# olivesgatech/R3D

Hardware: AMD Instinct MI355X
Metric: training clips/sec (RGB+Depth fusion, DARai) at 1/2/4/8 GPUs; effective-rank match (higher is better)
Workload: dtype f32 (depth products: bf16x3 split on the bf16 matrix cores, fp32 accumulate)

## Files before the change

include/r3d_hip.h:

```cpp
#ifndef R3D_HIP_H
#define R3D_HIP_H

#include <stdint.h>

#ifdef __cplusplus
extern "C" {
#endif

#define R3D_ABI_VERSION 2

#define R3D_OK 0
#define R3D_EINVAL (-1)
#define R3D_EALIGN (-2)
#define R3D_ENORCCL (-3)
#define R3D_ERCCL_BASE (-100)

int r3d_abi_version(void);
int r3d_build_info(char* buf, int cap);

int r3d_allreduce_flat(float* buf, int64_t count, void* comm, void* stream);

#define R3D_GEMM_NT 0
#define R3D_GEMM_NN 1
#define R3D_GEMM_TN 2
// ... 256 lines not shown
    const float* w_head; const float* b_head; int n_head;
    float* t3; float* m3; float* r3; float* tgtF; float* mF; float* rF; float* out; int ld_out; int H;
    const float* seg; int ld_seg; const int64_t* past_label; const int64_t* target; const float* target_dur;
    int B, S, Q, K, pad_idx, exclude_idx; const float* dur_den; float grad_scale;
    float* d_seg; int ld_dseg; float* d_out; int ld_dout; float* loss_out; int64_t* counts; int64_t* tick_a; int64_t* tick_b;
    const uint8_t* drop; float drop_scale; float* dx; float* dx2; float* wsF; float* ws3;
    int defer_finalize;
} r3d_tail_losses_args;
int r3d_decoder_tail_losses_supported(int H, int n_head, int Q, int rows);
int r3d_decoder_tail_losses(const r3d_tail_losses_args* a, float* ws, void* stream);

typedef struct r3d_decoder_chain_args {
    const float* caq; const float* cakv; const int64_t* key_label; float* p_ca; const uint8_t* drop_ca; float* ca_o;
    const float* wo; const float* bo; const uint8_t* drop_d2; const float* t1; float* t2_pre; const float* g2; const float* be2;
    float* t2; float* m2; float* r2; const float* w1; const float* b1; const uint8_t* drop_ff; float* ff1;
    const float* w2; const float* b2; const uint8_t* drop_d3; float* t3_pre;
    const float* d_t3pre; const float* d_ff2; float* d_ff1; float* d_t2pre; float* d_cap; float* d_cao; float* d_caq;
    float* d_cakv; float* part_d2;
    float drop_scale;
    int32_t pad_idx, B, S, H, Q, heads, phases;
    uint64_t* timeline;
    const uint16_t* pl_wo; const uint16_t* pl_w1; const uint16_t* pl_w2; const uint16_t* pl_w2_t; const uint16_t* pl_w1_t;
    const uint16_t* pl_wo_t;
} r3d_decoder_chain_args;
int r3d_decoder_chain_supported(int H, int Q, int heads, int S);
int r3d_decoder_chain(const r3d_decoder_chain_args* d, const r3d_tail_losses_args* tail, float* ws, void* stream);

int r3d_adamw_flat(float* p, const float* g, float* m, float* v, int64_t n, const float* lr, const int64_t* step,
                   float beta1, float beta2, float eps, float weight_decay, float grad_scale, void* stream);
int r3d_adamw_flat_dropout(float* p, const float* g, float* m, float* v, int64_t n, const float* lr, const int64_t* step,
                           float beta1, float beta2, float eps, float weight_decay, float grad_scale, uint8_t* mask,
                           int64_t n_mask, float p_drop, uint64_t seed, const int64_t* offset, void* stream);
typedef struct r3d_loss_finalize_job {
    const float* part; int32_t B, S, Q, has_seg;
    const float* dur_den;
    float* loss_out; int64_t* counts;
    double* acc_loss; int64_t* acc_counts;
} r3d_loss_finalize_job;
int r3d_losses_finalize(const r3d_loss_finalize_job* job, void* stream);
int r3d_adamw_flat_fin(float* p, const float* g, float* m, float* v, int64_t n, const float* lr, const int64_t* step,
                       float beta1, float beta2, float eps, float weight_decay, float grad_scale,
                       const r3d_loss_finalize_job* fin, void* stream);
int r3d_adamw_flat_dropout_fin(float* p, const float* g, float* m, float* v, int64_t n, const float* lr, const int64_t* step,
                               float beta1, float beta2, float eps, float weight_decay, float grad_scale, uint8_t* mask,
                               int64_t n_mask, float p_drop, uint64_t seed, const int64_t* offset,
                               const r3d_loss_finalize_job* fin, void* stream);
int r3d_adamw_2d(float* p, const float* g, float* m, float* v, int rows, int cols, int ld, const float* lr,
                 const int64_t* step, float beta1, float beta2, float eps, float weight_decay, float grad_scale, void* stream);
// ... 53 lines not shown
```

r3d_amd/_lib.py:

```python
import ctypes as C
import os

HERE = os.path.dirname(os.path.abspath(__file__))
LIB_PATH = os.path.join(HERE, "_build", "libr3d_hip.so")
ABI_VERSION = 2

c_float_p = C.c_void_p


class GemmDesc(C.Structure):
    _fields_ = [
        ("A", C.c_void_p), ("B", C.c_void_p), ("C", C.c_void_p),
        ("layout", C.c_int32), ("M", C.c_int32), ("N", C.c_int32), ("K", C.c_int32),
        ("lda", C.c_int32), ("ldb", C.c_int32), ("ldc", C.c_int32),
        ("a_add", C.c_void_p), ("a_add_mod", C.c_int32), ("a_add_ld", C.c_int32), ("a_row_xor", C.c_int32),
        ("b_add", C.c_void_p), ("b_add_mod", C.c_int32), ("b_add_ld", C.c_int32),
        ("bias", C.c_void_p),
        ("pre_out", C.c_void_p), ("ldpre", C.c_int32),
        ("act", C.c_int32),
        ("drop_mask", C.c_void_p), ("lddrop", C.c_int32), ("drop_scale", C.c_float),
        ("aux", C.c_void_p), ("ldaux", C.c_int32), ("mul", C.c_int32),
        ("res1", C.c_void_p), ("ldr1", C.c_int32),
        ("res2", C.c_void_p), ("ldr2", C.c_int32),
        ("alpha", C.c_float), ("accumulate", C.c_int32),
# ... 45 lines not shown


class PlaneJob(C.Structure):
    _fields_ = [("src", C.c_void_p), ("dst", C.c_void_p), ("ld", C.c_int32), ("N", C.c_int32), ("K", C.c_int32),
                ("transposed", C.c_int32), ("first_block", C.c_int32), ("pad_", C.c_int32)]


class FuserChainBwdArgs(C.Structure):
    _PTRS = ("d_cakv d_seg d_extra wkv wseg x3 mf rf gf w2 u w1 x1 m2 r2 g2 wproj wv x0 m1 r1 g1n drop_x0 m_rgb m_dep rgb "
             "dep_pre mean_d rstd_d lnd_g lnd_b d_fused d_x3 d_u d_h2 d_x1 d_v d_h1 d_rgb_pre d_dep_pre part_nf part_n2 "
             "part_n1 part_dep d_caq d_t1_res wq t1_pre m1d r1d g1d drop_d1 w_out sa_qkv p_sa drop_sa w_in caqin t1pre_out "
             "sap sao saqkv sain part_d1").split()
    _PLANES = "pl_wkv_t pl_wseg_t pl_w2_t pl_w1_t pl_wproj_t pl_wv_t".split()
    _fields_ = ([(n, C.c_void_p) for n in _PTRS] + [("drop_scale", C.c_float)] +
                [(n, C.c_int32) for n in "N S K H add_xres B Q heads".split()] + [("timeline", C.c_void_p)] +
                [(n, C.c_void_p) for n in _PLANES])


class DecoderChainArgs(C.Structure):
    _PTRS = ("caq cakv key_label p_ca drop_ca ca_o wo bo drop_d2 t1 t2_pre g2 be2 t2 m2 r2 w1 b1 drop_ff ff1 w2 b2 drop_d3 "
             "t3_pre d_t3pre d_ff2 d_ff1 d_t2pre d_cap d_cao d_caq d_cakv part_d2").split()
    _fields_ = ([(n, C.c_void_p) for n in _PTRS] + [("drop_scale", C.c_float)] +
                [(n, C.c_int32) for n in "pad_idx B S H Q heads phases".split()] + [("timeline", C.c_void_p)] +
                [(n, C.c_void_p) for n in "pl_wo pl_w1 pl_w2 pl_w2_t pl_w1_t pl_wo_t".split()])


class MhaJob(C.Structure):
    _fields_ = [("q", C.c_void_p), ("ldq", C.c_int32), ("k", C.c_void_p), ("ldk", C.c_int32), ("v", C.c_void_p),
                ("ldv", C.c_int32), ("key_padding_mask", C.c_void_p), ("key_label", C.c_void_p), ("pad_idx", C.c_int32),
                ("probs", C.c_void_p), ("drop_mask", C.c_void_p), ("drop_scale", C.c_float), ("o", C.c_void_p),
                ("ldo", C.c_int32), ("B", C.c_int32), ("heads", C.c_int32), ("Lq", C.c_int32), ("Lk", C.c_int32),
                ("dh", C.c_int32)]


class MhaBwdJob(C.Structure):
    _fields_ = [("q", C.c_void_p), ("ldq", C.c_int32), ("k", C.c_void_p), ("ldk", C.c_int32), ("v", C.c_void_p),
                ("ldv", C.c_int32), ("probs", C.c_void_p), ("drop_mask", C.c_void_p), ("drop_scale", C.c_float),
                ("d_o", C.c_void_p), ("lddo", C.c_int32), ("dq", C.c_void_p), ("lddq", C.c_int32), ("dk", C.c_void_p),
                ("lddk", C.c_int32), ("dv", C.c_void_p), ("lddv", C.c_int32), ("B", C.c_int32), ("heads", C.c_int32),
                ("Lq", C.c_int32), ("Lk", C.c_int32), ("dh", C.c_int32)]


class RowsumJob(C.Structure):
    _fields_ = [("src1", C.c_void_p), ("src2", C.c_void_p), ("dst", C.c_void_p), ("ld1", C.c_int32), ("ld2", C.c_int32),
                ("ldd", C.c_int32), ("rows", C.c_int32), ("cols", C.c_int32), ("mod", C.c_int32)]


# ... 36 lines not shown
    "r3d_build_info": ([C.c_char_p, _I], C.c_int),
    "r3d_allreduce_flat": ([_P, _L, _P, _P], C.c_int),
    "r3d_gemm_f32": ([C.POINTER(GemmDesc), _P], C.c_int),
    "r3d_splitk_reduce": ([C.POINTER(GemmDesc), _P], C.c_int),
    "r3d_gemm_partial_floats": ([C.c_int32, C.c_int32, C.c_int32], C.c_int64),
    "r3d_gemm_plan": ([C.POINTER(GemmDesc)], C.c_int),
    "r3d_gemm_grouped_prepare": ([C.POINTER(GemmDesc), _I, _I, C.POINTER(C.c_int32)], C.c_int),
    "r3d_gemm_grouped_launch": ([_P, _P, C.POINTER(C.c_int32), _I, _I, _I, _I, _P], C.c_int),
    "r3d_gemm_ln_supported": ([_I, _I, _I], C.c_int),
    "r3d_gemm_ln_fwd": ([_P, _I, _I, _P], C.c_int),
    "r3d_fuser_chain_supported": ([_I, _I, _I, _I, _I, _I], C.c_int),
    "r3d_fuser_chain_fwd": ([_P, _P], C.c_int),
    "r3d_fuser_chain_bwd": ([_P, _P], C.c_int),
    "r3d_weight_plane_elems": ([_I, _I], C.c_int64),
    "r3d_weight_planes": ([_P, _I, _I, _P], C.c_int),
    "r3d_token_exchange3_fwd": ([_P, _P, _P, _P, _P, _F, _P, _I, _I, _P], C.c_int),
    "r3d_token_exchange3_bwd": ([_P, _P, _P, _F, _P, _P, _P, _I, _I, _P], C.c_int),
    "r3d_attn3_fwd": ([_P, _P, _P, _I, _I, _I, _P], C.c_int),
    "r3d_attn3_bwd": ([_P, _P, _P, _I, _I, _I, _P], C.c_int),
    "r3d_triple_mean_fwd": ([_P, _P, _I, _I, _P], C.c_int),
    "r3d_triple_mean_bwd": ([_P, _P, _I, _I, _P], C.c_int),
    "r3d_decoder_chain_supported": ([_I, _I, _I, _I], C.c_int),
    "r3d_decoder_chain": ([_P, _P, _P, _P], C.c_int),
    "r3d_gemm_ln_mha_supported": ([_I, _I, _I, _I], C.c_int),
    "r3d_gemm_ln_mha_fwd": ([_P, _I, _I, _P, _P], C.c_int),
    "r3d_layernorm_fwd_multi": ([_P, _I, _P], C.c_int),
    "r3d_layernorm_bwd_multi": ([_P, _I, _P], C.c_int),
    "r3d_layernorm_bwd_multi_mha": ([_P, _I, _P, _P], C.c_int),
    "r3d_layernorm_bwd_finalize_batched": ([_P, _I, _I, _P], C.c_int),
    "r3d_layernorm_fwd": ([_P, _I, _I, _P, _P, _P, _P, _P, _I, _P, _P, _P, _I, _I, _I, _P], C.c_int),
    "r3d_layernorm_bwd_ws_floats": ([_I, _I], C.c_int64),
    "r3d_add_rowbcast": ([_P, _I, _P, _I, _I, _P, _I, _I, _I, _P], C.c_int),
    "r3d_layernorm_bwd": ([_P, _I, _I, _P, _I, _P, _I, _P, _P, _P, _P, _I, _P, _I, _P, _I, _P, _I, _P, _I, _P, _I, _F,
                           _P, _P, _P, _I, _I, _I, _P], C.c_int),
    "r3d_layernorm_bwd_finalize": ([_P, _I, _I, _P, _P, _P], C.c_int),
    "r3d_colsum_ws_floats": ([_I, _I], C.c_int64),
    "r3d_colsum": ([_P, _I, _I, _I, _P, _P, _I, _P], C.c_int),
    "r3d_rowmod_sum": ([_P, _I, _I, _I, _I, _P, _I, _I, _P], C.c_int),
    "r3d_rowmod_sum_batched": ([_P, _I, _I, _I, _P], C.c_int),
    "r3d_tick": ([_P, _P, _P], C.c_int),
    "r3d_colabssum": ([_P, _I, _I, _I, _P, _P], C.c_int),
    "r3d_token_select": ([_P, _P, _D, _I, _I, _I, _P, _P, _P, _P], C.c_int),
    "r3d_token_exchange_fwd": ([_P, _P, _P, _P, _P, _P, _F, _I, _I, _P], C.c_int),
    "r3d_token_exchange_bwd": ([_P, _P, _P, _P, _P, _F, _P, _P, _I, _I, _P], C.c_int),
    "r3d_mha_core_fwd": ([_P, _I, _P, _I, _P, _I, _P, _P, _I, _P, _P, _F, _P, _I, _I, _I, _I, _I, _I, _P], C.c_int),
    "r3d_mha_core_bwd": ([_P, _I, _P, _I, _P, _I, _P, _P, _F, _P, _I, _P, _I, _P, _I, _P, _I, _I, _I, _I, _I, _I, _P],
# ... 107 lines not shown
```

r3d_amd/csrc/decoder_chain.hip:

```cpp
#include "chain_bf3.h"
#include "mha_small.h"
#include "losses_dev.h"

namespace r3d {

constexpr int kDcBufA = 0;
constexpr int kDcBufB = kDcBufA + kFcRows * kFcP1;
constexpr int kDcBufF = kDcBufB + kFcRows * kFcP1;
constexpr int kDcWl = kDcBufF + kFcRows * kFcP4;
constexpr int kDcWlWave = 128 * kFbWP;
constexpr int kDcRed = kDcWl + 8 * kDcWlWave;
constexpr int kDcLdsFloats = kDcRed + 2 * 2 * 8 * kFcRows;
constexpr int kDcLdsBytes = kDcLdsFloats * 4;
static_assert(16 * kFcWP <= kDcWlWave && mha_small_lds_floats(16, 8) <= kDcWlWave && mha_small_bwd_lds_floats(16, 8) <= kDcWlWave,
              "wave region");
static_assert(kDcLdsBytes + (2 * 8 * (kTLHeads + 8) + 8 * 4 * 128 + 64) * 4 <= 160 * 1024, "LDS (dynamic + the tail's static arrays)");

typedef r3d_decoder_chain_args DcArgs;

__device__ __forceinline__ void dc_stage_rows(float* buf, const float* src, int row0, int tid) {
    const int r = tid >> 5, c4 = tid & 31;
    const f32x4 z = {0.f, 0.f, 0.f, 0.f};
    const f32x4 v = *reinterpret_cast<const f32x4*>(src + (size_t)(row0 + (r & 7)) * kFcH + 4 * c4);
    *reinterpret_cast<f32x4*>(buf + r * kFcP1 + 4 * c4) = r < 8 ? v : z;
// ... 540 lines not shown
    __shared__ float red[8][4][128];
    __shared__ int is_last;
    const int lane = threadIdx.x & 63, wave = threadIdx.x >> 6;
    if ((int)blockIdx.x < D.B) {
        const int b = (int)blockIdx.x;
        if (D.phases & 1) dc_fwd(D, b, lds);
        R3D_CHAIN_MARK(D.timeline, b == 0, 6);
        if (D.phases & 2) {
            __syncthreads();
            tail_clip_body(t, a, part, b, lg, dl, red);
        }
        R3D_CHAIN_MARK(D.timeline, b == 0, 7);
        if (D.phases & 4) {
            __syncthreads();
            dc_bwd(D, b, lds);
        }
    } else if (D.phases & 2) {
        const int u = ((int)blockIdx.x - D.B) * 8 + wave;
        if (u < a.B * a.S) losses_unit(a, part, u, lane);
    }
    if (D.phases & 2) tail_losses_finish(t, a, part, arrivals, &is_last);
}

}

using namespace r3d;

R3D_EXPORT int r3d_decoder_tail_losses_supported(int H, int n_head, int Q, int rows);

R3D_EXPORT int r3d_decoder_chain_supported(int H, int Q, int heads, int S) {
    return (H == kFcH && Q == 8 && heads == 8 && S > 0 && S <= 64) ? 1 : 0;
}

R3D_EXPORT int r3d_decoder_chain(const r3d_decoder_chain_args* d, const r3d_tail_losses_args* tail, float* ws, void* stream) {
    R3D_REQUIRE(d && (d->phases & 7) && !(d->phases & ~7));
    R3D_REQUIRE(r3d_decoder_chain_supported(d->H, d->Q, d->heads, d->S) && d->B > 0);
    R3D_REQUIRE(d->caq && d->cakv && d->p_ca && d->wo && d->w1 && d->w2 && d->t2_pre && d->m2 && d->r2 && d->g2 && d->ff1);
    if (d->phases & 1)
        R3D_REQUIRE(d->ca_o && d->bo && d->t1 && d->be2 && d->t2 && d->b1 && d->b2 && d->t3_pre);
    if (d->phases & 4)
        R3D_REQUIRE(d->d_t3pre && d->d_ff2 && d->d_ff1 && d->d_t2pre && d->d_cap && d->d_cao && d->d_caq && d->d_cakv && d->part_d2);
    const void* al[] = {d->caq, d->cakv, d->wo, d->w1, d->w2, d->ca_o, d->d_ff2, d->d_cao, d->d_cakv};
    for (const void* p : al)
        if (p && !r3d_aligned16(p)) return R3D_EALIGN;
    r3d_tail_losses_args t{};
    LossArgs a{};
    int grid = d->B;
    unsigned* arrivals = nullptr;
    if (d->phases & 2) {
        R3D_REQUIRE(tail && ws);
        t = *tail;
        R3D_REQUIRE(t.x && t.g3 && t.b3 && t.gF && t.bF && t.w_head && t.b_head && t.t3 && t.m3 && t.r3 && t.tgtF && t.mF && t.rF);
        R3D_REQUIRE(t.out && t.seg && t.past_label && t.target && t.target_dur && t.d_seg && t.d_out && t.loss_out && t.counts);
        R3D_REQUIRE(t.dx && t.dx2 && t.wsF && t.ws3);
        R3D_REQUIRE(t.B == d->B && t.S == d->S && t.Q == d->Q && t.H == d->H && t.K > 0 && t.n_head == t.K + 1);
        R3D_REQUIRE(t.ld_out >= t.n_head && t.ld_dout >= t.n_head && t.ld_seg >= t.K && t.ld_dseg >= t.K);
        if (!r3d_decoder_tail_losses_supported(t.H, t.n_head, t.Q, t.B * t.Q)) return R3D_EINVAL;
        if (!r3d_aligned16(ws)) return R3D_EALIGN;
        if (d->phases & 1) R3D_REQUIRE(t.x == d->t3_pre);
        if (d->phases & 4) R3D_REQUIRE(t.dx == d->d_t3pre && t.dx2 == d->d_ff2);
        a = LossArgs{t.seg, t.ld_seg, t.out, t.ld_out, t.out + t.K, t.ld_out, t.past_label, t.target, t.target_dur, t.B, t.S, t.Q,
                     t.K, t.pad_idx, t.exclude_idx, 0, t.dur_den, t.grad_scale, t.d_seg, t.ld_dseg, t.d_out, t.ld_dout,
                     t.d_out + t.K, t.ld_dout, t.loss_out, t.counts, t.tick_a, t.tick_b};
        const int units = t.B * t.S + t.B * t.Q + t.B;
        grid = t.B + r3d_cdiv(t.B * t.S, 8);
        arrivals = reinterpret_cast<unsigned*>(ws + 4 * (size_t)units);
    }
    if (d->pl_wo) {
        R3D_REQUIRE(d->pl_w1 && d->pl_w2 && d->pl_w2_t && d->pl_w1_t && d->pl_wo_t);
        hipError_t e3 = hipFuncSetAttribute((const void*)decoder_chain_bf3_kernel, hipFuncAttributeMaxDynamicSharedMemorySize,
                                            kD3LdsBytes);
        if (e3 != hipSuccess) return (int)e3;
        hipLaunchKernelGGL(decoder_chain_bf3_kernel, dim3(grid), dim3(512), (size_t)kD3LdsBytes, (hipStream_t)stream, *d, t, a, ws,
                           arrivals);
        R3D_LAUNCH_CHECK();
        return R3D_OK;
    }
    hipError_t e = hipFuncSetAttribute((const void*)decoder_chain_kernel, hipFuncAttributeMaxDynamicSharedMemorySize, kDcLdsBytes);
    if (e != hipSuccess) return (int)e;
    hipLaunchKernelGGL(decoder_chain_kernel, dim3(grid), dim3(512), (size_t)kDcLdsBytes, (hipStream_t)stream, *d, t, a, ws, arrivals);
    R3D_LAUNCH_CHECK();
    return R3D_OK;
}
```

r3d_amd/csrc/mha_small.h:

```cpp
#pragma once
#include "common.h"

namespace r3d {

struct MhaArgs {
    const float* q; int ldq; const float* k; int ldk; const float* v; int ldv;
    const uint8_t* kpm;
    const int64_t* key_label; int pad_idx;
    float* probs;
    const uint8_t* drop; float drop_scale;
    float* o; int ldo;
    const float* d_o; int lddo;
    float* dq; int lddq; float* dk; int lddk; float* dv; int lddv;
    int B, heads, Lq, Lk, dh; float scale;
};

constexpr int mha_small_lds_floats(int DH, int LQ) { return LQ * DH + LQ * 64 + 64 * (DH + 1); }

template <bool WG> __device__ __forceinline__ void mha_unit_sync() {
    if (WG) __syncthreads();
    else __builtin_amdgcn_wave_barrier();
}

template <int DH, int LQ, bool WG>
// ... 34 lines not shown
    for (int t = 0; t < DH / 4; ++t) {
        vc[lane * (DH + 1) + 4 * t + 0] = v4[t].x; vc[lane * (DH + 1) + 4 * t + 1] = v4[t].y;
        vc[lane * (DH + 1) + 4 * t + 2] = v4[t].z; vc[lane * (DH + 1) + 4 * t + 3] = v4[t].w;
    }
    mha_unit_sync<WG>();
    float keep[LQ];
#pragma unroll
    for (int i = 0; i < LQ; ++i) keep[i] = has_drop ? a.drop_scale * (float)kraw[i] : 1.f;
    const bool masked = lane >= Lk || (has_kpm && kpm_raw != 0) || (has_lab && lab_raw == (int64_t)a.pad_idx);
    float p[LQ];
#pragma unroll
    for (int i = 0; i < LQ; ++i) {
        float s = 0.f;
#pragma unroll
        for (int t = 0; t < DH / 4; ++t) {
            const float4 q4 = *reinterpret_cast<const float4*>(qs + i * DH + 4 * t);
            s += q4.x * k4[t].x + q4.y * k4[t].y + q4.z * k4[t].z + q4.w * k4[t].w;
        }
        s = masked ? -INFINITY : s * a.scale;
        const float m = wave_max(s);
        const float e = expf(s - m);
        const float sum = wave_sum(e);
        p[i] = e / sum;
        if (lane < Lk) a.probs[pbase + (size_t)i * Lk + lane] = p[i];
        sc[i * 64 + lane] = lane < Lk ? p[i] * keep[i] : 0.f;
    }
    mha_unit_sync<WG>();
#pragma unroll
    for (int t = 0; t < (LQ * DH + 63) / 64; ++t) {
        const int e = lane + 64 * t;
        if (e < LQ * DH) {
            const int i = e / DH, d = e % DH;
            float s = 0.f;
            for (int r = 0; r < Lk; ++r) s += sc[i * 64 + r] * vc[r * (DH + 1) + d];
            a.o[((size_t)b * LQ + i) * a.ldo + h * DH + d] = s;
        }
    }
}

constexpr int mha_small_bwd_lds_floats(int DH, int LQ) { return 2 * LQ * DH + LQ * 64 + 64 * (DH + 1); }

template <int DH, int LQ, bool WG>
__device__ __forceinline__ void mha_bwd_small_unit(const MhaArgs& a, const int unit, float* lds) {
    float* qs = lds;
    float* dos = lds + LQ * DH;
    float* ds = dos + LQ * DH;
    float* kc = ds + LQ * 64;
// ... 91 lines not shown
```

r3d_amd/engine.py:

```python
import math

import torch

from . import ops
from ._lib import GEMM_NT, GEMM_NN, GEMM_TN

LIVE_PREFIXES = ("input_embed.", "depth_projection.", "depth_layernorm.", "pos_embedding", "query_embed.",
                 "fuser.blocks.", "fuser.norm.", "transformer.decoder.", "fc_seg.", "fc.", "fc_len.")
EXCLUDE_CLASS_IDX = 47
DROP_P = 0.1


BN_LIVE_PREFIXES = ("fuser.alpha", "fuser.bn_rgb.", "fuser.bn_depth.")
VARY_LIVE_PREFIXES = ("fuser.alpha",)
PLAIN_LIVE_PREFIXES = ("fuser.modality_token",)


def is_live(name):
    return name.startswith(LIVE_PREFIXES)


BWD_BF3_MAX_K = 32


# ... 211 lines not shown
        self.bn = hasattr(module.fuser, "bn_rgb")
        self.vary = (not self.bn) and hasattr(module.fuser, "alpha")
        self.plain = getattr(type(module.fuser), "r3d_fuser_kind", None) == "plain"
        check_engine_shape(self.H, self.heads, self.Q, self.bn, self.vary, self.plain)
        self.max_pos_len = module.pos_embedding.shape[1]
        extra = (BN_LIVE_PREFIXES if self.bn else (VARY_LIVE_PREFIXES if self.vary else
                                                   (PLAIN_LIVE_PREFIXES if self.plain else ())))
        self.arena = ParamArena(list(module.named_parameters()), self.device, extra)
        self.ws = ops.GemmWorkspace(self.device)
        self._sel = {}
        self.ws_side = ops.GemmWorkspace(self.device)
        self.side = torch.cuda.Stream(self.device)
        self.side2 = torch.cuda.Stream(self.device)
        self.ws_side2 = ops.GemmWorkspace(self.device)
        self.auto_side_stream = True
        self.use_side_stream = False
        self.use_fused_decoder = False
        self.use_fused_tail = True
        self.defer_tail = False
        self.use_paired_launches = True
        self.use_gemm_ln = True
        self.use_fuser_chain = True
        self.use_decoder_chain = True
        self.chain_bf3 = True
        self._planes = None
        self.overlap_planes = False
        self.overlap_param_tail = False
        self.ride_planes = True
        self._planes_rode = False
        self.fuse_depth_adamw = True
        self.pair_embeddings = True
        self._planes_forked = False
        self._tail_pending = False
        self._overlap_tail_now = False
        self.defer_loss_reduce = False
        self.loss_acc = None
        self.fold_rowsums = True
        self.ride_attention = True
        self.ride_attention_bwd = False
        self.split_k4h = False
        self.depth_prec = 1
        self.use_fused_embed = not (self.bn or self.vary)
        self.dropout_enabled = bool(getattr(module, "r3d_dropout_enabled", True))
        self.erank_weight = 0.0
        self.erank_warm_start = False
        self.erank_max_sweeps = 16
# ... 385 lines not shown
        key = ("dec_chain", bool(drop), bf3)
        if bf3 and not (self.use_fuser_chain and self._chain_shape_ok(w)):
            self._planes_refresh()
        if key not in w.tables:
            pls = self.chain_planes() if bf3 else None
            dpl = None
            if pls is not None:
                dpl = dict(pl_wo=pls.ptr("pl_dec_wo"), pl_w1=pls.ptr("pl_dec_w1"), pl_w2=pls.ptr("pl_dec_w2"),
                           pl_w2_t=pls.ptr("pl_dec_w2_t"), pl_w1_t=pls.ptr("pl_dec_w1_t"), pl_wo_t=pls.ptr("pl_dec_wo_t"))
            a, H = self.arena, self.H
            c, pl = w.layers[0], "transformer.decoder.layers.0."
            dk = (lambda k: w.drop[k]) if drop else (lambda k: None)
            gl = w.glayers[0] if hasattr(w, "glayers") else None
            g = (lambda k: gl[k]) if gl is not None else (lambda k: None)
            w.tables[key] = ops.DecoderChain(
                caq=c["caq"], cakv=c["cakv"], p_ca=c["p_ca"], drop_ca=dk("ca_p0"), ca_o=c["ca_o"],
                wo=a.p(pl + "multihead_attn.out_proj.weight"), bo=a.p(pl + "multihead_attn.out_proj.bias"), drop_d2=dk("d2_0"),
                t1=c["t1"], t2_pre=c["t2_pre"], g2=a.p(pl + "norm2.weight"), be2=a.p(pl + "norm2.bias"), t2=c["t2"], m2=c["m2"],
                r2=c["r2"], w1=a.p(pl + "linear1.weight"), b1=a.p(pl + "linear1.bias"), drop_ff=dk("ff_0"), ff1=c["ff1"],
                w2=a.p(pl + "linear2.weight"), b2=a.p(pl + "linear2.bias"), drop_d3=dk("d3_0"), t3_pre=c["t3_pre"],
                d_t3pre=g("t3pre"), d_ff2=g("ff2"), d_ff1=g("ff1"), d_t2pre=g("t2pre"), d_cap=g("cap"), d_cao=g("cao"),
                d_caq=g("caq"), d_cakv=g("cakv"), part_d2=w.lnp["d2_0"] if gl is not None else None,
                drop_scale=1.0 / (1.0 - DROP_P), pad_idx=self.pad_idx, B=w.B, S=w.S, H=H, Q=self.Q, heads=self.heads, planes=dpl)
        return w.tables[key]

    def _gln(self, rows, K):
        return self.use_gemm_ln and ops.gemm_ln_supported(rows, K, self.H)

    def _forward_paired(self, w, fw, dm, dsc, drop, wv, pre, qpos, pos):
        a, H, Q, S, B, BQ, heads, dh = self.arena, self.H, self.Q, w.S, w.B, w.BQ, self.heads, self.dh
        c, pl = w.layers[0], "transformer.decoder.layers.0."
        if self._chain_ok(w):
            bf3 = bool(self.chain_bf3)
            key = ("fwd_chain", bool(drop), bf3)
            if bf3:
                self._planes_refresh()
            if key not in w.tables:
                pls = self.chain_planes() if bf3 else None
                wi, bi = a.p(pl + "multihead_attn.in_proj_weight"), a.p(pl + "multihead_attn.in_proj_bias")
                w.tables[key] = ops.FuserChainFwd(
                    x0=w.x0, h1=w.h1, wv=wv, wproj=a.p(pre + "attn.proj.weight"), bproj=a.p(pre + "attn.proj.bias"),
                    g2=a.p(pre + "norm2.weight"), be2=a.p(pre + "norm2.bias"), w1=a.p(pre + "mlp.mlp.0.weight"),
                    b1=a.p(pre + "mlp.mlp.0.bias"), w2=a.p(pre + "mlp.mlp.2.weight"), b2=a.p(pre + "mlp.mlp.2.bias"),
                    gf=a.p("fuser.norm.weight"), bef=a.p("fuser.norm.bias"), pos=pos.contiguous(), wkv=wi[H:], bkv=bi[H:],
                    wseg=a.p("fc_seg.weight"), bseg=a.p("fc_seg.bias"), vsw=w.vsw, x1=w.x1, h2=w.h2, m2=w.m2, r2=w.r2, u=w.u,
                    f1=w.f1, x3=w.x3, y=w.y, mf=w.mf, rf=w.rf, fused=w.fused, seg=w.seg, cakv=c["cakv"],
# ... 769 lines not shown
```

r3d_amd/ops.py:

```python
import ctypes as C

import torch

from . import _lib
from ._lib import GemmDesc, GEMM_NT, GEMM_NN, GEMM_TN, check


def _stream():
    return C.c_void_p(torch.cuda.current_stream().cuda_stream)


def _pv(t):
    return None if t is None else t.data_ptr()


def _p(t):
    if t is None:
        return None
    assert t.is_cuda, "r3d_amd kernels take device tensors only"
    return C.c_void_p(t.data_ptr())


def _f32(t, name="tensor"):
    assert t.dtype == torch.float32 and t.is_cuda, f"{name} must be a float32 device tensor"
# ... 392 lines not shown
            for name in FuserChainBwdArgs._PLANES:
                setattr(a, name, planes[name])
        for name in FuserChainBwdArgs._PTRS:
            v = t.pop(name, None)
            if v is None:
                assert name in opt, name
                continue
            assert v.is_cuda and v.is_contiguous(), name
            assert v.dtype == (torch.uint8 if name.startswith("drop_") else torch.float32), name
            setattr(a, name, v.data_ptr())
        assert not t, t.keys()
        for k, v in dims.items():
            setattr(a, k, int(v))
        self.args = a

    def launch(self):
        check(_lib.load().r3d_fuser_chain_bwd(C.byref(self.args), _stream()), "r3d_fuser_chain_bwd")


def decoder_chain_supported(H, Q, heads, S):
    return bool(_lib.load().r3d_decoder_chain_supported(H, Q, heads, S))


class DecoderChain:

    def __init__(self, **t):
        from ._lib import DecoderChainArgs
        a = DecoderChainArgs()
        dims = {k: t.pop(k) for k in ("pad_idx", "B", "S", "H", "Q", "heads")}
        a.drop_scale = float(t.pop("drop_scale", 1.0))
        opt = {"key_label", "drop_ca", "drop_d2", "drop_ff", "drop_d3", "d_t3pre", "d_ff2", "d_ff1", "d_t2pre", "d_cap", "d_cao",
               "d_caq", "d_cakv", "part_d2"}
        planes = t.pop("planes", None)
        if planes is not None:
            for name in ("pl_wo", "pl_w1", "pl_w2", "pl_w2_t", "pl_w1_t", "pl_wo_t"):
                setattr(a, name, planes[name])
        for name in DecoderChainArgs._PTRS:
            v = t.pop(name, None)
            if v is None:
                assert name in opt, name
                continue
            assert v.is_cuda and v.is_contiguous(), name
            want = torch.uint8 if name.startswith("drop_") else (torch.int64 if name == "key_label" else torch.float32)
            assert v.dtype == want, name
            setattr(a, name, v.data_ptr())
        assert not t, t.keys()
        for k, v in dims.items():
            setattr(a, k, int(v))
        self.args = a

    def launch(self, phases, key_label=None, tail=None, ws=None):
        a = self.args
        a.phases = int(phases)
        a.key_label = None if key_label is None else key_label.data_ptr()
        check(_lib.load().r3d_decoder_chain(C.byref(a), C.byref(tail) if tail is not None else None, _p(ws), _stream()),
              "r3d_decoder_chain")


def layernorm_bwd_multi(jobs, mha=None):
    from ._lib import LnBwdJob
    arr = (LnBwdJob * len(jobs))()
    for i, j in enumerate(jobs):
        rows, H = j["x"].shape
        a = arr[i]
        g = lambda k: j.get(k)
        a.dy, a.lddy, a.pair_in = j["dy"].data_ptr(), _ld(j["dy"]), 1 if g("pair_in") else 0
        a.dy2, a.lddy2 = _pv(g("dy2")), _ld(g("dy2")) if g("dy2") is not None else 0
        a.x, a.ldx, a.mean, a.rstd = j["x"].data_ptr(), _ld(j["x"]), j["mean"].data_ptr(), j["rstd"].data_ptr()
        a.gamma, a.beta, a.relu = j["gamma"].data_ptr(), j["beta"].data_ptr(), 1 if g("relu") else 0
        a.add1, a.ldadd1 = _pv(g("add1")), _ld(g("add1")) if g("add1") is not None else 0
        a.add2, a.ldadd2 = _pv(g("add2")), _ld(g("add2")) if g("add2") is not None else 0
        a.dx, a.lddx = j["dx"].data_ptr(), _ld(j["dx"])
        a.dx2, a.lddx2 = _pv(g("dx2")), _ld(g("dx2")) if g("dx2") is not None else 0
        a.drop_mask, a.lddrop = _pv(g("drop_mask")), _ld(g("drop_mask")) if g("drop_mask") is not None else 0
        a.drop_scale = g("drop_scale") or 1.0
        a.dgamma, a.dbeta, a.ws = j["dgamma"].data_ptr(), j["dbeta"].data_ptr(), j["partial"].data_ptr()
# ... 594 lines not shown
```

Baseline: 44120.

## Split decoder chain across four workgroups per clip with atomic arrival handoff

```diff
diff --git a/include/r3d_hip.h b/include/r3d_hip.h
--- a/include/r3d_hip.h
+++ b/include/r3d_hip.h
@@ -302,8 +302,10 @@
     uint64_t* timeline;
     const uint16_t* pl_wo; const uint16_t* pl_w1; const uint16_t* pl_w2; const uint16_t* pl_w2_t; const uint16_t* pl_w1_t;
     const uint16_t* pl_wo_t;
+    float* split_ws; int32_t groups;
 } r3d_decoder_chain_args;
 int r3d_decoder_chain_supported(int H, int Q, int heads, int S);
+int64_t r3d_decoder_chain_ws_floats(int B);
 int r3d_decoder_chain(const r3d_decoder_chain_args* d, const r3d_tail_losses_args* tail, float* ws, void* stream);
 
 int r3d_adamw_flat(float* p, const float* g, float* m, float* v, int64_t n, const float* lr, const int64_t* step,
diff --git a/r3d_amd/_lib.py b/r3d_amd/_lib.py
--- a/r3d_amd/_lib.py
+++ b/r3d_amd/_lib.py
@@ -91,7 +91,8 @@
              "t3_pre d_t3pre d_ff2 d_ff1 d_t2pre d_cap d_cao d_caq d_cakv part_d2").split()
     _fields_ = ([(n, C.c_void_p) for n in _PTRS] + [("drop_scale", C.c_float)] +
                 [(n, C.c_int32) for n in "pad_idx B S H Q heads phases".split()] + [("timeline", C.c_void_p)] +
-                [(n, C.c_void_p) for n in "pl_wo pl_w1 pl_w2 pl_w2_t pl_w1_t pl_wo_t".split()])
+                [(n, C.c_void_p) for n in "pl_wo pl_w1 pl_w2 pl_w2_t pl_w1_t pl_wo_t".split()] +
+                [("split_ws", C.c_void_p), ("groups", C.c_int32)])
 
 
 class MhaJob(C.Structure):
@@ -174,6 +175,7 @@
     "r3d_triple_mean_bwd": ([_P, _P, _I, _I, _P], C.c_int),
     "r3d_decoder_chain_supported": ([_I, _I, _I, _I], C.c_int),
     "r3d_decoder_chain": ([_P, _P, _P, _P], C.c_int),
+    "r3d_decoder_chain_ws_floats": ([_I], C.c_int64),
     "r3d_gemm_ln_mha_supported": ([_I, _I, _I, _I], C.c_int),
     "r3d_gemm_ln_mha_fwd": ([_P, _I, _I, _P, _P], C.c_int),
     "r3d_layernorm_fwd_multi": ([_P, _I, _P], C.c_int),
diff --git a/r3d_amd/csrc/decoder_chain.hip b/r3d_amd/csrc/decoder_chain.hip
--- a/r3d_amd/csrc/decoder_chain.hip
+++ b/r3d_amd/csrc/decoder_chain.hip
@@ -586,6 +586,291 @@
     if (D.phases & 2) tail_losses_finish(t, a, part, arrivals, &is_last);
 }
 
+
+constexpr int kDsG = 4;
+constexpr int kDsSlab = 8 * kFcH;
+static_assert(kDsG * 8 * 16 == 4 * kFcH, "a group's slice is 8 tiles of 16: one per wave");
+
+__host__ __device__ inline unsigned* ds_counters(float* ws, int B) { return reinterpret_cast<unsigned*>(ws + (size_t)B * kDsG * kDsSlab); }
+
+__device__ __forceinline__ void split_wt_store(float* p, float v) { __hip_atomic_store(p, v, __ATOMIC_RELAXED, __HIP_MEMORY_SCOPE_AGENT); }
+
+__device__ __forceinline__ bool ds_arrive(unsigned* cnt, int* flag) {
+    asm volatile("s_waitcnt vmcnt(0)" ::: "memory");
+    __syncthreads();
+    if (threadIdx.x == 0) {
+        const bool last = __hip_atomic_fetch_add(cnt, 1u, __ATOMIC_RELAXED, __HIP_MEMORY_SCOPE_AGENT) == (unsigned)(kDsG - 1);
+        if (last) {
+            __builtin_amdgcn_fence(__ATOMIC_ACQUIRE, "agent");
+            asm volatile("s_waitcnt vmcnt(0)" ::: "memory");
+            __hip_atomic_store(cnt, 0u, __ATOMIC_RELAXED, __HIP_MEMORY_SCOPE_AGENT);
+        }
+        *flag = last ? 1 : 0;
+    }
+    __syncthreads();
+    return *flag != 0;
+}
+
+__device__ __forceinline__ void ds3_stage_rows4(unsigned short* img, const float* src, int row0, int tid) {
+    const f32x4 z = {0.f, 0.f, 0.f, 0.f};
+#pragma unroll
+    for (int j = 0; j < 4; ++j) {
+        const int e = tid + 512 * j, r = e >> 7, c4 = e & 127;
+        const f32x4 v = *reinterpret_cast<const f32x4*>(src + (size_t)(row0 + (r & 7)) * (4 * kFcH) + 4 * c4);
+        bf3_store4(img, kD3P4, r, 4 * c4, r < 8 ? v : z);
+    }
+}
+
+__device__ __forceinline__ bool ds3_fwd(const DcArgs& D, const int b, const int g, float* lds, int* flag) {
+    const int tid = threadIdx.x, lane = tid & 63, wave = tid >> 6;
+    const int li = lane & 15, q = lane >> 4;
+    unsigned short* img = reinterpret_cast<unsigned short*>(lds);
+    unsigned short* imgA = img + kD3ImgA;
+    unsigned short* imgB = img + kD3ImgB;
+    unsigned short* imgF = img + kD3ImgF;
+    float* scr = reinterpret_cast<float*>(reinterpret_cast<unsigned char*>(lds) + kD3ScrBytes) + wave * kD3ScrWave;
+    float (*red)[8][kFcRows] = reinterpret_cast<float (*)[8][kFcRows]>(reinterpret_cast<unsigned char*>(lds) + kD3RedBytes);
+    constexpr int H = kFcH;
+    const int row0 = b * 8;
+    const int c = wave * 16 + li;
+    const int tf = 8 * g + wave;
+    const int cu = tf * 16 + li;
+    const bool live = q < 2;
+    const bool mark = b == 0 && g == 0;
+    const f32x4 zero = {0.f, 0.f, 0.f, 0.f};
+    R3D_CHAIN_MARK(D.timeline, mark, 0);
+    Bf3B b0, b1, b2;
+    bf3_bload<4>(b0, D.pl_wo, 4, wave, 0, lane);
+    bf3_bload<4>(b1, D.pl_w1, 4, tf, 0, lane);
+    bf3_bload<4>(b2, D.pl_w2, 16, wave, 0, lane);
+    const FcMaskSrc md2(D.drop_d2, D.g2, H), md3(D.drop_d3, D.g2, H), mff(D.drop_ff, D.g2, 4 * H);
+    float t1v[4];
+    uint8_t kb2[4], kb3[4], kbf[4];
+#pragma unroll
+    for (int i = 0; i < 4; ++i) {
+        const size_t r = (size_t)(row0 + ((4 * q + i) & 7));
+        t1v[i] = D.t1[r * H + c];
+        kb2[i] = md2.raw(r, c);
+        kb3[i] = md3.raw(r, c);
+        kbf[i] = mff.raw(r, cu);
+    }
+    const float b_o = D.bo[c], g2 = D.g2[c], be2 = D.be2[c], b_2 = D.b2[c], b_1 = D.b1[cu];
+    R3D_CHAIN_MARK(D.timeline, mark, 1);
+    float* cao = g == 0 ? D.ca_o : D.split_ws + ((size_t)b * kDsG + g) * kDsSlab - (size_t)row0 * H;
+    {
+        MhaArgs m{};
+        m.q = D.caq; m.ldq = H; m.k = D.cakv; m.ldk = 2 * H; m.v = D.cakv + H; m.ldv = 2 * H;
+        m.key_label = D.key_label; m.pad_idx = D.pad_idx; m.probs = g == 0 ? D.p_ca : nullptr; m.drop = D.drop_ca;
+        m.drop_scale = D.drop_scale; m.o = cao; m.ldo = H; m.B = D.B; m.heads = 8; m.Lq = 8; m.Lk = D.S; m.dh = 16;
+        m.scale = 0.25f;
+        mha_fwd_small_unit<16, 8, false>(m, b * 8 + wave, scr);
+    }
+    R3D_CHAIN_MARK(D.timeline, mark, 2);
+    __syncthreads();
+    dc3_stage_rows(imgA, cao, row0, tid);
+    __syncthreads();
+    R3D_CHAIN_MARK(D.timeline, mark, 3);
+    f32x4 acc0 = zero, acc1 = zero;
+    bf3_chunk<4>(imgA, kD3P1, li, q, 0, b0, acc0, acc1);
+    __builtin_amdgcn_sched_barrier(0);
+    bf3_bload<4>(b0, D.pl_w2, 16, wave, 4, lane);
+    __builtin_amdgcn_sched_barrier(0);
+    float t2p[4], mean[4], rstd[4], t2v[4];
+#pragma unroll
+    for (int i = 0; i < 4; ++i) {
+        t2p[i] = ((acc0[i] + acc1[i]) + b_o) * md2.keep(kb2[i], D.drop_scale) + t1v[i];
+        if (live && g == 0) D.t2_pre[(size_t)(row0 + 4 * q + i) * H + c] = t2p[i];
+    }
+    fc_layernorm(t2p, red, wave, li, q, mean, rstd);
+#pragma unroll
+    for (int i = 0; i < 4; ++i) {
+        t2v[i] = (t2p[i] - mean[i]) * rstd[i] * g2 + be2;
+        const int r = 4 * q + i;
+        if (live && g == 0) {
+            D.t2[(size_t)(row0 + r) * H + c] = t2v[i];
+            if (wave == 0 && li == 0) { D.m2[row0 + r] = mean[i]; D.r2[row0 + r] = rstd[i]; }
+        }
+        bf3_store1(imgB, kD3P1, r, c, live ? t2v[i] : 0.f);
+    }
+    __syncthreads();
+    R3D_CHAIN_MARK(D.timeline, mark, 4);
+    acc0 = zero; acc1 = zero;
+    bf3_chunk<4>(imgB, kD3P1, li, q, 0, b1, acc0, acc1);
+    __builtin_amdgcn_sched_barrier(0);
+    bf3_bload<4>(b1, D.pl_w2, 16, wave, 8, lane);
+    __builtin_amdgcn_sched_barrier(0);
+    if (live) {
+#pragma unroll
+        for (int i = 0; i < 4; ++i)
+            split_wt_store(D.ff1 + (size_t)(row0 + 4 * q + i) * (4 * H) + cu,
+                        fmaxf((acc0[i] + acc1[i]) + b_1, 0.f) * mff.keep(kbf[i], D.drop_scale));
+    }
+    R3D_CHAIN_MARK(D.timeline, mark, 5);
+    if (!ds_arrive(ds_counters(D.split_ws, D.B) + b, flag)) return false;
+    R3D_CHAIN_MARK(D.timeline, b == 0, 8);
+    ds3_stage_rows4(imgF, D.ff1, row0, tid);
+    __syncthreads();
+    R3D_CHAIN_MARK(D.timeline, b == 0, 9);
+    acc0 = zero; acc1 = zero;
+    bf3_chunk<4>(imgF, kD3P4, li, q, 0, b2, acc0, acc1);
+    __builtin_amdgcn_sched_barrier(0);
+    bf3_bload<4>(b2, D.pl_w2, 16, wave, 12, lane);
+    __builtin_amdgcn_sched_barrier(0);
+    bf3_chunk<4>(imgF, kD3P4, li, q, 4, b0, acc0, acc1);
+    bf3_chunk<4>(imgF, kD3P4, li, q, 8, b1, acc0, acc1);
+    bf3_chunk<4>(imgF, kD3P4, li, q, 12, b2, acc0, acc1);
+    if (live) {
+#pragma unroll
+        for (int i = 0; i < 4; ++i)
+            D.t3_pre[(size_t)(row0 + 4 * q + i) * H + c] =
+                ((acc0[i] + acc1[i]) + b_2) * md3.keep(kb3[i], D.drop_scale) + t2v[i];
+    }
+    return true;
+}
+
+__device__ __forceinline__ void ds3_bwd(const DcArgs& D, const int b, const int g, float* lds, int* flag) {
+    const int tid = threadIdx.x, lane = tid & 63, wave = tid >> 6;
+    const int li = lane & 15, q = lane >> 4;
+    unsigned short* img = reinterpret_cast<unsigned short*>(lds);
+    unsigned short* imgA = img + kD3ImgA;
+    unsigned short* imgF = img + kD3ImgF;
+    float* scr = reinterpret_cast<float*>(reinterpret_cast<unsigned char*>(lds) + kD3ScrBytes) + wave * kD3ScrWave;
+    float* redA = reinterpret_cast<float*>(reinterpret_cast<unsigned char*>(lds) + kD3RedBytes);
+    constexpr int H = kFcH;
+    const int row0 = b * 8;
+    const int c = wave * 16 + li;
+    const int tf = 8 * g + wave;
+    const int cu = tf * 16 + li;
+    const bool live = q < 2;
+    const bool mark = b == 0 && g == 0;
+    const f32x4 zero = {0.f, 0.f, 0.f, 0.f};
+    R3D_CHAIN_MARK(D.timeline, mark, 16);
+    Bf3B b0, b1, b2;
+    bf3_bload<4>(b0, D.pl_w2_t, 4, tf, 0, lane);
+    bf3_bload<4>(b1, D.pl_w1_t, 16, wave, 0, lane);
+    bf3_bload<4>(b2, D.pl_w1_t, 16, wave, 4, lane);
+    dc3_stage_rows(imgA, D.d_ff2, row0, tid);
+    const FcMaskSrc md2(D.drop_d2, D.g2, H), mff(D.drop_ff, D.g2, 4 * H);
+    float ffv[4], res[4], t2pv[4], m2v[4], r2v[4];
+    uint8_t kb2[4], kbf[4];
+#pragma unroll
+    for (int i = 0; i < 4; ++i) {
+        const size_t r = (size_t)(row0 + ((4 * q + i) & 7));
+        ffv[i] = D.ff1[r * (4 * H) + cu];
+        kbf[i] = mff.raw(r, cu);
+        res[i] = D.d_t3pre[r * H + c];
+        t2pv[i] = D.t2_pre[r * H + c];
+        m2v[i] = D.m2[r]; r2v[i] = D.r2[r];
+        kb2[i] = md2.raw(r, c);
+    }
+    const float g2 = D.g2[c];
+    __syncthreads();
+    R3D_CHAIN_MARK(D.timeline, mark, 17);
+    f32x4 acc0 = zero, acc1 = zero;
+    bf3_chunk<4>(imgA, kD3P1, li, q, 0, b0, acc0, acc1);
+    __builtin_amdgcn_sched_barrier(0);
+    bf3_bload<4>(b0, D.pl_w1_t, 16, wave, 8, lane);
+    __builtin_amdgcn_sched_barrier(0);
+    if (live) {
+#pragma unroll
+        for (int i = 0; i < 4; ++i)
+            split_wt_store(D.d_ff1 + (size_t)(row0 + 4 * q + i) * (4 * H) + cu,
+                        ffv[i] > 0.f ? (acc0[i] + acc1[i]) * mff.keep(kbf[i], D.drop_scale) : 0.f);
+    }
+    R3D_CHAIN_MARK(D.timeline, mark, 18);
+    if (!ds_arrive(ds_counters(D.split_ws, D.B) + D.B + b, flag)) return;
+    R3D_CHAIN_MARK(D.timeline, b == 0, 19);
+    ds3_stage_rows4(imgF, D.d_ff1, row0, tid);
+    __syncthreads();
+    R3D_CHAIN_MARK(D.timeline, b == 0, 20);
+    acc0 = zero; acc1 = zero;
+    bf3_chunk<4>(imgF, kD3P4, li, q, 0, b1, acc0, acc1);
+    __builtin_amdgcn_sched_barrier(0);
+    bf3_bload<4>(b1, D.pl_w1_t, 16, wave, 12, lane);
+    __builtin_amdgcn_sched_barrier(0);
+    bf3_chunk<4>(imgF, kD3P4, li, q, 4, b2, acc0, acc1);
+    __builtin_amdgcn_sched_barrier(0);
+    bf3_bload<4>(b2, D.pl_wo_t, 4, wave, 0, lane);
+    __builtin_amdgcn_sched_barrier(0);
+    bf3_chunk<4>(imgF, kD3P4, li, q, 8, b0, acc0, acc1);
+    bf3_chunk<4>(imgF, kD3P4, li, q, 12, b1, acc0, acc1);
+    {
+        float d[4], xh[4], gg[4], gx[4], s1v[4], s2v[4];
+#pragma unroll
+        for (int i = 0; i < 4; ++i) {
+            d[i] = live ? (acc0[i] + acc1[i]) + res[i] : 0.f;
+            xh[i] = (t2pv[i] - m2v[i]) * r2v[i];
+            gg[i] = d[i] * g2;
+            gx[i] = gg[i] * xh[i];
+        }
+        if (live) {
+            float* pp = D.part_d2 + (size_t)(2 * b + q) * (2 * H);
+            pp[c] = (d[0] * xh[0] + d[1] * xh[1]) + (d[2] * xh[2] + d[3] * xh[3]);
+            pp[H + c] = (d[0] + d[1]) + (d[2] + d[3]);
+        }
+        fb_rowsum2<4>(gg, gx, redA, wave, li, q, s1v, s2v);
+#pragma unroll
+        for (int i = 0; i < 4; ++i) {
+            const float o = r2v[i] * (gg[i] - s1v[i] - xh[i] * s2v[i]);
+            const size_t e = (size_t)(row0 + 4 * q + i) * H + c;
+            const float ok = o * md2.keep(kb2[i], D.drop_scale);
+            if (live) { D.d_t2pre[e] = o; D.d_cap[e] = ok; }
+            bf3_store1(imgA, kD3P1, 4 * q + i, c, live ? ok : 0.f);
+        }
+    }
+    __syncthreads();
+    R3D_CHAIN_MARK(D.timeline, b == 0, 21);
+    acc0 = zero; acc1 = zero;
+    bf3_chunk<4>(imgA, kD3P1, li, q, 0, b2, acc0, acc1);
+    if (live) {
+#pragma unroll
+        for (int i = 0; i < 4; ++i) D.d_cao[(size_t)(row0 + 4 * q + i) * H + c] = acc0[i] + acc1[i];
+    }
+    R3D_CHAIN_MARK(D.timeline, b == 0, 22);
+    __syncthreads();
+    {
+        MhaArgs m{};
+        m.q = D.caq; m.ldq = H; m.k = D.cakv; m.ldk = 2 * H; m.v = D.cakv + H; m.ldv = 2 * H;
+        m.probs = D.p_ca; m.drop = D.drop_ca; m.drop_scale = D.drop_scale; m.d_o = D.d_cao; m.lddo = H;
+        m.dq = D.d_caq; m.lddq = H; m.dk = D.d_cakv; m.lddk = 2 * H; m.dv = D.d_cakv + H; m.lddv = 2 * H;
+        m.B = D.B; m.heads = 8; m.Lq = 8; m.Lk = D.S; m.dh = 16; m.scale = 0.25f;
+        mha_bwd_small_unit<16, 8, false>(m, b * 8 + wave, scr);
+    }
+    R3D_CHAIN_MARK(D.timeline, b == 0, 23);
+}
+
+__global__ __launch_bounds__(512) void decoder_chain_split_fwd_kernel(const DcArgs D, const r3d_tail_losses_args t, const LossArgs a,
+                                                                      float* part, unsigned* arrivals) {
+    extern __shared__ __attribute__((aligned(16))) float lds[];
+    __shared__ float lg[8][kTLHeads + 8];
+    __shared__ float dl[8][kTLHeads + 8];
+    __shared__ float red[8][4][128];
+    __shared__ int is_last;
+    if (threadIdx.x >= 256) __builtin_amdgcn_s_setprio(0); else __builtin_amdgcn_s_setprio(2);
+    const int lane = threadIdx.x & 63, wave = threadIdx.x >> 6;
+    if ((int)blockIdx.x < kDsG * D.B) {
+        const int b = (int)blockIdx.x / kDsG, g = (int)blockIdx.x % kDsG;
+        const bool own = (D.phases & 1) ? ds3_fwd(D, b, g, lds, &is_last) : g == 0;
+        R3D_CHAIN_MARK(D.timeline, b == 0 && own, 6);
+        if (own && (D.phases & 2)) {
+            __syncthreads();
+            tail_clip_body(t, a, part, b, lg, dl, red);
+        }
+        R3D_CHAIN_MARK(D.timeline, b == 0 && own, 7);
+    } else if (D.phases & 2) {
+        const int u = ((int)blockIdx.x - kDsG * D.B) * 8 + wave;
+        if (u < a.B * a.S) losses_unit(a, part, u, lane);
+    }
+    if (D.phases & 2) tail_losses_finish(t, a, part, arrivals, &is_last);
+}
+
+__global__ __launch_bounds__(512) void decoder_chain_split_bwd_kernel(const DcArgs D) {
+    extern __shared__ __attribute__((aligned(16))) float lds[];
+    __shared__ int is_last;
+    if (threadIdx.x >= 256) __builtin_amdgcn_s_setprio(0); else __builtin_amdgcn_s_setprio(2);
+    ds3_bwd(D, (int)blockIdx.x / kDsG, (int)blockIdx.x % kDsG, lds, &is_last);
+}
+
 }
 
 using namespace r3d;
@@ -596,8 +881,13 @@
     return (H == kFcH && Q == 8 && heads == 8 && S > 0 && S <= 64) ? 1 : 0;
 }
 
+R3D_EXPORT int64_t r3d_decoder_chain_ws_floats(int B) {
+    return B > 0 ? (int64_t)B * kDsG * kDsSlab + 4 * r3d_cdiv(2 * B, 4) : 0;
+}
+
 R3D_EXPORT int r3d_decoder_chain(const r3d_decoder_chain_args* d, const r3d_tail_losses_args* tail, float* ws, void* stream) {
     R3D_REQUIRE(d && (d->phases & 7) && !(d->phases & ~7));
+    R3D_REQUIRE(d->groups >= 0 && (d->groups <= 1 || d->groups == kDsG));
     R3D_REQUIRE(r3d_decoder_chain_supported(d->H, d->Q, d->heads, d->S) && d->B > 0);
     R3D_REQUIRE(d->caq && d->cakv && d->p_ca && d->wo && d->w1 && d->w2 && d->t2_pre && d->m2 && d->r2 && d->g2 && d->ff1);
     if (d->phases & 1)
@@ -630,6 +920,32 @@
         grid = t.B + r3d_cdiv(t.B * t.S, 8);
         arrivals = reinterpret_cast<unsigned*>(ws + 4 * (size_t)units);
     }
+    if (d->pl_wo && d->groups == kDsG) {
+        R3D_REQUIRE(d->pl_w1 && d->pl_w2 && d->pl_w2_t && d->pl_w1_t && d->pl_wo_t && d->split_ws);
+        if (!r3d_aligned16(d->split_ws)) return R3D_EALIGN;
+        if (d->phases & 3) {
+            hipError_t e3 = hipFuncSetAttribute((const void*)decoder_chain_split_fwd_kernel,
+                                                hipFuncAttributeMaxDynamicSharedMemorySize, kD3LdsBytes);
+            if (e3 != hipSuccess) return (int)e3;
+            r3d_decoder_chain_args f = *d;
+            f.phases = d->phases & 3;
+            const int gf = kDsG * d->B + grid - d->B;
+            hipLaunchKernelGGL(decoder_chain_split_fwd_kernel, dim3(gf), dim3(512), (size_t)kD3LdsBytes, (hipStream_t)stream, f,
+                               t, a, ws, arrivals);
+            R3D_LAUNCH_CHECK();
+        }
+        if (d->phases & 4) {
+            hipError_t e3 = hipFuncSetAttribute((const void*)decoder_chain_split_bwd_kernel,
+                                                hipFuncAttributeMaxDynamicSharedMemorySize, kD3LdsBytes);
+            if (e3 != hipSuccess) return (int)e3;
+            r3d_decoder_chain_args bk = *d;
+            bk.phases = 4;
+            hipLaunchKernelGGL(decoder_chain_split_bwd_kernel, dim3(kDsG * d->B), dim3(512), (size_t)kD3LdsBytes,
+                               (hipStream_t)stream, bk);
+            R3D_LAUNCH_CHECK();
+        }
+        return R3D_OK;
+    }
     if (d->pl_wo) {
         R3D_REQUIRE(d->pl_w1 && d->pl_w2 && d->pl_w2_t && d->pl_w1_t && d->pl_wo_t);
         hipError_t e3 = hipFuncSetAttribute((const void*)decoder_chain_bf3_kernel, hipFuncAttributeMaxDynamicSharedMemorySize,
diff --git a/r3d_amd/csrc/mha_small.h b/r3d_amd/csrc/mha_small.h
--- a/r3d_amd/csrc/mha_small.h
+++ b/r3d_amd/csrc/mha_small.h
@@ -80,7 +80,7 @@
         const float e = expf(s - m);
         const float sum = wave_sum(e);
         p[i] = e / sum;
-        if (lane < Lk) a.probs[pbase + (size_t)i * Lk + lane] = p[i];
+        if (a.probs && lane < Lk) a.probs[pbase + (size_t)i * Lk + lane] = p[i];
         sc[i * 64 + lane] = lane < Lk ? p[i] * keep[i] : 0.f;
     }
     mha_unit_sync<WG>();
diff --git a/r3d_amd/engine.py b/r3d_amd/engine.py
--- a/r3d_amd/engine.py
+++ b/r3d_amd/engine.py
@@ -257,6 +257,7 @@
         self.use_gemm_ln = True
         self.use_fuser_chain = True
         self.use_decoder_chain = True
+        self.decoder_chain_groups = 4
         self.chain_bf3 = True
         self._planes = None
         self.overlap_planes = False
@@ -688,6 +689,7 @@
                 d_t3pre=g("t3pre"), d_ff2=g("ff2"), d_ff1=g("ff1"), d_t2pre=g("t2pre"), d_cap=g("cap"), d_cao=g("cao"),
                 d_caq=g("caq"), d_cakv=g("cakv"), part_d2=w.lnp["d2_0"] if gl is not None else None,
                 drop_scale=1.0 / (1.0 - DROP_P), pad_idx=self.pad_idx, B=w.B, S=w.S, H=H, Q=self.Q, heads=self.heads, planes=dpl)
+        w.tables[key].groups = int(self.decoder_chain_groups)
         return w.tables[key]
 
     def _gln(self, rows, K):
diff --git a/r3d_amd/ops.py b/r3d_amd/ops.py
--- a/r3d_amd/ops.py
+++ b/r3d_amd/ops.py
@@ -438,6 +438,10 @@
     return bool(_lib.load().r3d_decoder_chain_supported(H, Q, heads, S))
 
 
+def decoder_chain_ws_floats(B):
+    return int(_lib.load().r3d_decoder_chain_ws_floats(B))
+
+
 class DecoderChain:
 
     def __init__(self, **t):
@@ -451,6 +455,7 @@
         if planes is not None:
             for name in ("pl_wo", "pl_w1", "pl_w2", "pl_w2_t", "pl_w1_t", "pl_wo_t"):
                 setattr(a, name, planes[name])
+        dev = t["caq"].device
         for name in DecoderChainArgs._PTRS:
             v = t.pop(name, None)
             if v is None:
@@ -463,11 +468,17 @@
         assert not t, t.keys()
         for k, v in dims.items():
             setattr(a, k, int(v))
+        self.split_ws = None
+        if planes is not None:
+            self.split_ws = torch.zeros(decoder_chain_ws_floats(a.B), dtype=torch.float32, device=dev)
+            a.split_ws = self.split_ws.data_ptr()
+        self.groups = 1
         self.args = a
 
     def launch(self, phases, key_label=None, tail=None, ws=None):
         a = self.args
         a.phases = int(phases)
+        a.groups = int(self.groups) if self.split_ws is not None else 1
         a.key_label = None if key_label is None else key_label.data_ptr()
         check(_lib.load().r3d_decoder_chain(C.byref(a), C.byref(tail) if tail is not None else None, _p(ws), _stream()),
               "r3d_decoder_chain")
```

Measured after the change: 44910 (median of 6 runs). 1.02x the previous value.
